# hellosunking/Microcket

Hardware: AMD Instinct MI355X
Metric: read-pairs/sec through sam2pairs+dedup (150 bp PE, hg38 names, SAM text resident in HBM) (higher is better)
Workload: dtype u8; 1 GPU; C2: 100 M 150 bp PE Micro-C read pairs, hg38, one MI355X -- 100000000 synthetic 150 bp PE read pairs per GPU, hg38 chromosome names, 1 lane(s), unc mode, sam=no, seed 20260105, one step = one pass over the whole resident data set + duplicate marking of the reported pairs on (chr1,pos1,chr2,pos2,strands) + per-chromosome-pair counts; preset=C2, pairs_per_gpu=100000001, sam_bytes_per_gpu=94584442002, block_groups=2097152, blocks=48, parallelism=shard1: independent read-group shards, no data-path collective

## Files before the change

### microcket_amd/build.py

```python
import os
import shutil
import subprocess
import sys

HERE = os.path.dirname(os.path.abspath(__file__))
ROOT = os.path.dirname(HERE)
CSRC = os.path.join(HERE, "csrc")
LIB = os.path.join(HERE, "libmkt_hip.so")
EXE = os.path.join(HERE, "bin", "sam2pairs")
ARCH = "gfx950"


def _newer(target, sources):
    if not os.path.exists(target):
        return True
    t = os.path.getmtime(target)
    return any(os.path.getmtime(s) > t for s in sources)


def _run(cmd, **kw):
    print("+", " ".join(cmd), flush=True)
    subprocess.check_call(cmd, **kw)


# ... 134 lines not shown


PAIRSCMP = os.path.join(HERE, "bin", "pairscmp")


def build_pairscmp(force=False):
    src = os.path.join(CSRC, "pairscmp_main.cpp")
    if force or _newer(PAIRSCMP, [src, LIB] + _headers()):
        os.makedirs(os.path.dirname(PAIRSCMP), exist_ok=True)
        _run(["g++", "-O2", "-std=c++17", "-Wall", src, "-o", PAIRSCMP, "-L" + HERE, "-lmkt_hip",
              "-Wl,-rpath,$ORIGIN/..", "-Wl,-rpath,/opt/rocm/lib", "-Wl,-rpath-link,/opt/rocm/lib"])
    return PAIRSCMP


PAIRSBGZ = os.path.join(HERE, "bin", "pairsbgz")


def build_pairsbgz(force=False):
    src = os.path.join(CSRC, "pairsbgz_main.cpp")
    if force or _newer(PAIRSBGZ, [src, LIB] + _headers()):
        os.makedirs(os.path.dirname(PAIRSBGZ), exist_ok=True)
        _run(["g++", "-O2", "-std=c++17", "-Wall", src, "-o", PAIRSBGZ, "-L" + HERE, "-lmkt_hip",
              "-Wl,-rpath,$ORIGIN/..", "-Wl,-rpath,/opt/rocm/lib", "-Wl,-rpath-link,/opt/rocm/lib"])
    return PAIRSBGZ


PAIRSGUNZIP = os.path.join(HERE, "bin", "pairsgunzip")


def build_pairsgunzip(force=False):
    src = os.path.join(CSRC, "pairsgunzip_main.cpp")
    if force or _newer(PAIRSGUNZIP, [src, LIB] + _headers()):
        os.makedirs(os.path.dirname(PAIRSGUNZIP), exist_ok=True)
        _run(["g++", "-O2", "-std=c++17", "-Wall", src, "-o", PAIRSGUNZIP, "-L" + HERE, "-lmkt_hip",
              "-Wl,-rpath,$ORIGIN/..", "-Wl,-rpath,/opt/rocm/lib", "-Wl,-rpath-link,/opt/rocm/lib"])
    return PAIRSGUNZIP


PAIRSQUERY = os.path.join(HERE, "bin", "pairsquery")


def build_pairsquery(force=False):
    src = os.path.join(CSRC, "pairsquery_main.cpp")
    if force or _newer(PAIRSQUERY, [src, LIB] + _headers()):
        os.makedirs(os.path.dirname(PAIRSQUERY), exist_ok=True)
        _run(["g++", "-O2", "-std=c++17", "-Wall", src, "-o", PAIRSQUERY, "-L" + HERE, "-lmkt_hip",
              "-Wl,-rpath,$ORIGIN/..", "-Wl,-rpath,/opt/rocm/lib", "-Wl,-rpath-link,/opt/rocm/lib"])
    return PAIRSQUERY


BAM2SAM = os.path.join(HERE, "bin", "bam2sam")


def build_bam2sam(force=False):
    src = os.path.join(CSRC, "bam2sam_main.cpp")
    if force or _newer(BAM2SAM, [src, LIB] + _headers()):
        os.makedirs(os.path.dirname(BAM2SAM), exist_ok=True)
        _run(["g++", "-O2", "-std=c++17", "-Wall", src, "-o", BAM2SAM, "-L" + HERE, "-lmkt_hip",
              "-Wl,-rpath,$ORIGIN/..", "-Wl,-rpath,/opt/rocm/lib", "-Wl,-rpath-link,/opt/rocm/lib"])
    return BAM2SAM


MAKESTAT = os.path.join(HERE, "bin", "makestat")


def build_makestat(force=False):
    src = os.path.join(CSRC, "makestat_main.cpp")
    if force or _newer(MAKESTAT, [src]):
        os.makedirs(os.path.dirname(MAKESTAT), exist_ok=True)
        _run(["g++", "-O2", "-std=c++17", "-Wall", src, "-o", MAKESTAT])
    return MAKESTAT


def build_oracle():
    _run(["make", "-s", "-C", os.path.join(ROOT, "oracle")])


def build_emit_parts():
    out = os.path.join(ROOT, "tests", "host", "_build")
    os.makedirs(out, exist_ok=True)
    src = os.path.join(ROOT, "tests", "host", "emit_parts.cpp")
    made = []
    for name, extra in (("emit_parts", ()), ("emit_parts_san", ("-fsanitize=address,undefined", "-fno-sanitize-recover=all", "-fno-omit-frame-pointer"))):
        exe = os.path.join(out, name)
        if os.path.exists(src) and _newer(exe, [src] + _headers()):
            _run(["g++", "-O1", "-g", "-std=c++17", "-Wall", *extra, "-o", exe, src])
        made.append(exe)
    return made


def build_test_tools():
    out = os.path.join(ROOT, "tests", "host", "_build")
    os.makedirs(out, exist_ok=True)
    emul = os.path.join(out, "libmkt_emul.so")
    src = os.path.join(ROOT, "tests", "host", "tile_emul.cpp")
    if _newer(emul, [src] + _headers()):
        _run(["g++", "-O1", "-g", "-std=c++17", "-Wall", "-fPIC", "-shared", "-o", emul, src])
    dzc = os.path.join(out, "deflate_codes")
    dsrc = os.path.join(ROOT, "tests", "host", "deflate_codes.cpp")
    if os.path.exists(dsrc) and _newer(dzc, [dsrc, os.path.join(CSRC, "mkt_deflate_codes.h")]):
        _run(["g++", "-O1", "-g", "-std=c++17", "-Wall", "-o", dzc, dsrc])
    sth = os.path.join(out, "stitch_thresholds")
    tsrc = os.path.join(ROOT, "tests", "host", "stitch_thresholds.cpp")
    if os.path.exists(tsrc) and _newer(sth, [tsrc, os.path.join(CSRC, "mkt_stitch.h"), os.path.join(ROOT, "include", "mkt.h")]):
        _run(["g++", "-O1", "-g", "-std=c++17", "-Wall", "-o", sth, tsrc])
    dbc = os.path.join(out, "devbuf_check")
    bsrc = os.path.join(ROOT, "tests", "host", "devbuf_check.cpp")
    if os.path.exists(bsrc) and _newer(dbc, [bsrc, os.path.join(CSRC, "mkt_devbuf.h")]):
        _run([hipcc(), f"--offload-arch={ARCH}", "-O1", "-g", "-std=c++17", "-Wall", "-Wl,-rpath,/opt/rocm/lib", "-o", dbc, bsrc])
    vsrc = os.path.join(ROOT, "tests", "host", "viewpoint_host.cpp")
    for name, extra in (("viewpoint_host", ()), ("viewpoint_host_san", ("-fsanitize=address,undefined", "-fno-sanitize-recover=all", "-fno-omit-frame-pointer"))):
        vph = os.path.join(out, name)
        if os.path.exists(vsrc) and _newer(vph, [vsrc, os.path.join(CSRC, "mkt_viewpoint.h"), os.path.join(ROOT, "include", "mkt.h")]):
            _run(["g++", "-O1", "-g", "-std=c++17", "-Wall", *extra, "-o", vph, vsrc])
    csrc = os.path.join(ROOT, "tests", "host", "chunked_file.cpp")
    for name, extra in (("chunked_file", ()), ("chunked_file_san", ("-fsanitize=address,undefined", "-fno-sanitize-recover=all", "-fno-omit-frame-pointer"))):
        chf = os.path.join(out, name)
        if os.path.exists(csrc) and _newer(chf, [csrc, os.path.join(CSRC, "mkt_chunked_file.h")]):
            _run(["g++", "-O1", "-g", "-std=c++17", "-Wall", *extra, "-o", chf, csrc])
    psrc = os.path.join(ROOT, "tests", "host", "paircmp_host.cpp")
    for name, extra in (("paircmp_host", ()), ("paircmp_host_san", ("-fsanitize=address,undefined", "-fno-sanitize-recover=all", "-fno-omit-frame-pointer"))):
        pch = os.path.join(out, name)
        if os.path.exists(psrc) and _newer(pch, [psrc, os.path.join(CSRC, "mkt_paircmp.h"), os.path.join(ROOT, "include", "mkt.h")]):
            _run(["g++", "-O1", "-g", "-std=c++17", "-Wall", *extra, "-o", pch, psrc])
    xsrc = os.path.join(ROOT, "tests", "host", "px2_host.cpp")
    for name, extra in (("px2_host", ()), ("px2_host_san", ("-fsanitize=address,undefined", "-fno-sanitize-recover=all", "-fno-omit-frame-pointer"))):
        pxh = os.path.join(out, name)
        if os.path.exists(xsrc) and _newer(pxh, [xsrc, os.path.join(CSRC, "mkt_px2.h")]):
            _run(["g++", "-O1", "-g", "-std=c++17", "-Wall", *extra, "-o", pxh, xsrc])
    isrc = os.path.join(ROOT, "tests", "host", "inflate_host.cpp")
    for name, extra in (("inflate_host", ()), ("inflate_host_san", ("-fsanitize=address,undefined", "-fno-sanitize-recover=all", "-fno-omit-frame-pointer"))):
        ifh = os.path.join(out, name)
        if os.path.exists(isrc) and _newer(ifh, [isrc, os.path.join(CSRC, "mkt_inflate.h")]):
            _run(["g++", "-O1", "-g", "-std=c++17", "-Wall", *extra, "-o", ifh, isrc])
    qsrc = os.path.join(ROOT, "tests", "host", "pairsquery_host.cpp")
    for name, extra in (("pairsquery_host", ()), ("pairsquery_host_san", ("-fsanitize=address,undefined", "-fno-sanitize-recover=all", "-fno-omit-frame-pointer"))):
        pqh = os.path.join(out, name)
        if os.path.exists(qsrc) and _newer(pqh, [qsrc, os.path.join(CSRC, "mkt_px2query.h"), os.path.join(CSRC, "mkt_inflate.h")]):
            _run(["g++", "-O1", "-g", "-std=c++17", "-Wall", *extra, "-o", pqh, qsrc])
    bsrc2 = os.path.join(ROOT, "tests", "host", "bamtext_host.cpp")
    for name, extra in (("bamtext_host", ()), ("bamtext_host_san", ("-fsanitize=address,undefined", "-fno-sanitize-recover=all", "-fno-omit-frame-pointer"))):
        bth = os.path.join(out, name)
        if os.path.exists(bsrc2) and _newer(bth, [bsrc2, os.path.join(CSRC, "mkt_bamtext.h")]):
            _run(["g++", "-O1", "-g", "-std=c++17", "-Wall", *extra, "-o", bth, bsrc2])
    build_emit_parts()
    tout = os.path.join(ROOT, "tools", "_build")
    os.makedirs(tout, exist_ok=True)
    synth = os.path.join(tout, "synth_sam")
    ssrc = os.path.join(ROOT, "tools", "synth_sam.cpp")
    if _newer(synth, [ssrc, os.path.join(CSRC, "mkt_synth.h")]):
        _run(["g++", "-O2", "-std=c++17", "-Wall", "-o", synth, ssrc])


def build_all(force=False, extras=True):
    build_lib(force)
    build_exe(force)
    build_pairsort(force)
    build_krmdup(force)
    build_stitch(force)
    build_sam2bam(force)
    build_pairs2matrix(force)
    build_pairscmp(force)
    build_pairsbgz(force)
    build_pairsgunzip(force)
    build_pairsquery(force)
    build_bam2sam(force)
    build_makestat(force)
    if extras:
        build_oracle()
        build_test_tools()


if __name__ == "__main__":
    build_all(force="--force" in sys.argv, extras="--all" in sys.argv or True)
```

### microcket_amd/csrc/mkt_fast.h

```cpp
#pragma once
#include "mkt_tile.h"

namespace mkt {

#if defined(MKT_LEAN_GEOM)
constexpr int kLeanGeom[4] = {MKT_LEAN_GEOM};
constexpr int kLeanTile = kLeanGeom[0], kLeanHB = kLeanGeom[1], kLeanHF = kLeanGeom[2], kLeanLCAP = kLeanGeom[3];
#else
constexpr int kLeanTile = 49152, kLeanHB = 3072, kLeanHF = 4096, kLeanLCAP = 168;
#endif
constexpr int kMidTile = 32768, kMidHB = 2048, kMidHF = 3072, kMidLCAP = 160;
constexpr int kDenseTile = 16384, kDenseHB = 1024, kDenseHF = 2048, kDenseLCAP = 160;
constexpr int kLeanLinesTarget = 126;

constexpr double kLeanHaloBackLines = 7.5, kLeanHaloFwdLines = 8.75;
MKT_HD TileDims lean_dims(double avg) {
    if (avg < 48.0) avg = 48.0;
    if (avg > 4096.0) avg = 4096.0;
    auto r16 = [](double x) { return ((uint32_t)x + 15u) & ~15u; };
    TileDims d;
    d.hb = r16(kLeanHaloBackLines * avg); d.hf = r16(kLeanHaloFwdLines * avg);
    if (d.hb < 256u) d.hb = 256u;
    if (d.hb > (uint32_t)kLeanHB) d.hb = (uint32_t)kLeanHB;
    if (d.hf < 512u) d.hf = 512u;
// ... 17 lines not shown
    static constexpr int HCH = 8, HEADB = HCH * 16;
    static constexpr int HSTRIDE = HEADB + 4;
    static constexpr int HW = LCAP_ * HSTRIDE;
    static_assert(TILE_ % 16 == 0 && HB_ % 16 == 0 && HF_ % 16 == 0, "16-byte vector staging");
    static_assert(W < 65536, "window-relative offsets are 16 bit");
    static_assert(LCAP_ <= 255, "line / group ordinals are 8 bit");
    static_assert(LCAP_ * 132 < 65536, "head-store offsets are 16 bit");
};

enum { AB_LCAP = 1, AB_LONG, AB_TAB, AB_PREV_WS, AB_PREV_HEAD, AB_NO_PREV, AB_OPEN_GROUP, AB_LAST_LINE, AB_GCAP, AB_PAIR_BYTES, AB_SHORT_LINE };

constexpr uint8_t LB_EMIT = 8;

template <class Cfg>
struct FastState {
    alignas(16) uint8_t win[Cfg::HW + 16];
    struct Recs {
        struct { uint32_t pos[Cfg::LCAP], lclip[Cfg::LCAP], rclip[Cfg::LCAP], mappable[Cfg::LCAP], right0[Cfg::LCAP], left1[Cfg::LCAP], right1[Cfg::LCAP]; } f;
    } rc;
    uint16_t hv16[Cfg::LCAP];
    uint16_t off16[Cfg::LCAP];
    uint16_t goff[Cfg::LCAP];
    uint16_t flag[Cfg::LCAP];
    uint8_t qn_off[Cfg::LCAP], qn_len[Cfg::LCAP], rn_off[Cfg::LCAP], rn_len[Cfg::LCAP], segCnt[Cfg::LCAP], bits[Cfg::LCAP];
    union alignas(16) Phase {
        struct {
            uint64_t hitmap[Cfg::HMW + 1];
            alignas(8) uint16_t hmask[Cfg::LCAP][Cfg::HCH];
        } m;
        struct {
            uint32_t g_info[Cfg::LCAP], g_slen[Cfg::LCAP];
            uint32_t x_sam[Cfg::LCAP];
            uint16_t g_plen[Cfg::LCAP], x_pair[Cfg::LCAP];
            uint8_t x_grp[Cfg::LCAP], x_sc[Cfg::LCAP], x_emit[Cfg::LCAP], em_idx[Cfg::LCAP], g_slot[Cfg::LCAP];
            uint32_t l_posA[Cfg::GCAP], l_posB[Cfg::GCAP];
            uint16_t l_qa[Cfg::GCAP], l_ca[Cfg::GCAP], l_cb[Cfg::GCAP];
            uint16_t l_e0[Cfg::GCAP], l_e1[Cfg::GCAP], l_e2[Cfg::GCAP], l_e3[Cfg::GCAP];
            uint64_t l_litA[Cfg::GCAP][2], l_litB[Cfg::GCAP][2];
        } g;
    } u;
    uint64_t m_surv[4], m_eqp[4], m_r1[4], m_r2[4], m_start[4], m_emit[4];
    uint64_t cc[64];
    uint32_t NL, first_idx, end_idx, abn, last_line_end, nslot, c_t0, c_t1;
    uint32_t cnt[C_COUNT];
    TileSums sums, base;
    uint32_t region_pair0, region_sam0, region_id;
};

template <class Cfg> MKT_HD TileGeom fast_geom(uint32_t tile, uint32_t n) { return tile_geom(tile, n, cfg_dims<Cfg>()); }
template <class Cfg> MKT_HD TextView fast_view(const FastState<Cfg>& st, const uint8_t* text, uint32_t n, const TileGeom& G) {
    TextView tv;
    (void)G;
    tv.g = text; tv.n = n; tv.win = st.win; tv.w0 = 0; tv.wlen = Cfg::HW; tv.nlm = nullptr; tv.wsm = nullptr;
    return tv;
}
template <class Cfg> MKT_HD void fast_init(FastState<Cfg>& st, uint32_t k) { if (k < 64u) st.cc[k] = 0; }
template <class Cfg> MKT_HD uint32_t fast_chr_slot(FastState<Cfg>& st, ChrTab* tab, const TextView& tv, uint32_t off, uint32_t len, uint32_t* err) {
    static_assert(kChrSlots <= 8192, "slot in 13 bits");
    if (len == 0u || len > 6u) return chr_slot(tab, tv, off, len, err);
    const uint64_t name = ((uint64_t)win_load4(tv, off) | ((uint64_t)win_load4(tv, off + 4u) << 32)) & ((1ull << (8u * len)) - 1ull);
    const uint32_t idx = (uint32_t)((name * 0x9E3779B1ull) >> 30) & 63u;
    const uint64_t e0 = st.cc[idx], e1 = st.cc[idx ^ 1u];
    if ((e0 >> 63) && (e0 & 0xFFFFFFFFFFFFull) == name) return (uint32_t)(e0 >> 48) & 8191u;
    if ((e1 >> 63) && (e1 & 0xFFFFFFFFFFFFull) == name) return (uint32_t)(e1 >> 48) & 8191u;
    const uint32_t s = chr_slot(tab, tv, off, len, err);
    st.cc[(e0 >> 63) && !(e1 >> 63) ? (idx ^ 1u) : idx] = name | ((uint64_t)s << 48) | (1ull << 63);
    return s;
}
template <class Cfg> MKT_HD void fast_reset(FastState<Cfg>& st) {
    st.NL = 0; st.first_idx = 0; st.end_idx = 0; st.abn = 0; st.last_line_end = kUnknown; st.nslot = 0; st.c_t0 = 0; st.c_t1 = 0;
    for (int k = 0; k < 4; ++k) st.m_emit[k] = 0;
    st.region_pair0 = 0; st.region_sam0 = 0; st.region_id = 0;
    for (int k = 0; k < (int)C_COUNT; ++k) st.cnt[k] = 0;
}
template <class Cfg> MKT_HD uint32_t fast_nle(const FastState<Cfg>& st) {
    return (st.NL && (st.bits[st.NL - 1] & LB_CUT)) ? st.NL - 1u : st.NL;
}
template <class Cfg> MKT_HD uint32_t fast_line_end(const FastState<Cfg>& st, const TileGeom& G, uint32_t i) {
    return i + 1 < st.NL ? G.w0 + st.goff[i + 1] - 1u : st.last_line_end;
}

template <class Cfg> MKT_HD void fast_head_ws(const FastState<Cfg>& st, uint32_t i, uint64_t& ws0, uint64_t& ws1) {
    const uint64_t* row = reinterpret_cast<const uint64_t*>(st.u.m.hmask[i]);
    const uint64_t A = row[0], B = row[1];
    const uint32_t sh = (uint32_t)st.off16[i] - mul24(i, (uint32_t)Cfg::HSTRIDE);
    ws0 = sh ? ((A >> sh) | (B << (64u - sh))) : A;
    ws1 = B >> sh;
}
template <class Cfg> MKT_HD void fast_head_chunk_ref(FastState<Cfg>& st, const uint8_t* text, uint32_t n, const TileGeom& G, uint32_t i, uint32_t c) {
    const uint32_t r0 = 16u * ((uint32_t)st.hv16[i] + c);
    uint32_t m = 0;
    for (uint32_t b = 0; b < 16u; ++b) {
        const uint64_t g = (uint64_t)G.w0 + r0 + b;
        const uint8_t ch = g < n ? text[g] : 0;
        st.win[i * Cfg::HSTRIDE + 16u * c + b] = ch;
        if (g < n && ch <= 0x20u) m |= 1u << b;
    }
    st.u.m.hmask[i][c] = (uint16_t)m;
}

MKT_HD uint32_t nl_flags_exact(uint32_t x) {
    const uint32_t y = (x ^ 0x0A0A0A0Au), z = y & 0x7F7F7F7Fu;
    return ~((z + 0x7F7F7F7Fu) | y | 0x7F7F7F7Fu);
}
template <class Cfg> MKT_HD uint32_t fast_row_start(const FastState<Cfg>& st, const TileGeom& G, uint32_t i, bool* multi) {
    *multi = false;
    if (i == 0u && G.w0 == 0u) return 0u;
    const uint32_t* row = reinterpret_cast<const uint32_t*>(&st.win[mul24(i, (uint32_t)Cfg::HSTRIDE)]);
    const uint32_t f0 = nl_flags_exact(row[0]), f1 = nl_flags_exact(row[1]), f2 = nl_flags_exact(row[2]), f3 = nl_flags_exact(row[3]);
    const uint32_t m = (f0 >> 7) | (f1 >> 6) | (f2 >> 5) | (f3 >> 4);
    *multi = (m & (m - 1u)) != 0u;
    const uint32_t p = f0 ? (ctz32(f0) >> 3) : (f1 ? 4u + (ctz32(f1) >> 3) : (f2 ? 8u + (ctz32(f2) >> 3) : 12u + (ctz32(f3 | 0x80000000u) >> 3)));
    return p + 1u;
}

enum { LP_OK = 1, LP_NOREC = 2, LP_LONG = 0, LP_ODD = -1 };

MKT_HD uint32_t dec4(uint32_t w, bool& ok) {
    const uint32_t d = w ^ 0x30303030u;
    if (((d + 0x76767676u) | d) & 0x80808080u) ok = false;
    const uint32_t x = (d << 3) + (d << 1) + (d >> 8);
    return mul24(x & 0xFFu, 100u) + ((x >> 16) & 0xFFu);
}
MKT_HD uint32_t lean_uint4(const TextView& tv, uint32_t a, uint32_t len, bool& ok) {
    const uint32_t sh = 8u * (4u - len);
    const uint32_t w = (win_load4(tv, a) << sh) | (0x30303030u & ((1u << sh) - 1u));
    return dec4(w, ok);
}
MKT_HD uint32_t lean_uint12(const TextView& tv, uint32_t e, uint32_t len, bool& ok) {
    const uint32_t* w = reinterpret_cast<const uint32_t*>(tv.win);
    const uint32_t a = e - 12u, k = a >> 2, sh = a & 3u;
    const uint32_t q0 = w[k], q1 = w[k + 1], q2 = w[k + 2], q3 = w[k + 3];
    uint32_t x0, x1, x2;
#if defined(__HIP_DEVICE_COMPILE__)
    x0 = __builtin_amdgcn_alignbyte(q1, q0, sh); x1 = __builtin_amdgcn_alignbyte(q2, q1, sh); x2 = __builtin_amdgcn_alignbyte(q3, q2, sh);
#else
    x0 = sh ? ((q0 >> (8u * sh)) | (q1 << (32u - 8u * sh))) : q0;
    x1 = sh ? ((q1 >> (8u * sh)) | (q2 << (32u - 8u * sh))) : q1;
    x2 = sh ? ((q2 >> (8u * sh)) | (q3 << (32u - 8u * sh))) : q2;
#endif
    const uint32_t lead = 12u - len;
    const uint32_t n0 = lead < 4u ? lead : 4u, n1 = lead < 4u ? 0u : (lead < 8u ? lead - 4u : 4u), n2 = lead < 8u ? 0u : lead - 8u;
    const uint32_t m0 = n0 >= 4u ? 0xFFFFFFFFu : ((1u << (8u * n0)) - 1u), m1 = n1 >= 4u ? 0xFFFFFFFFu : ((1u << (8u * n1)) - 1u),
                   m2 = (1u << (8u * n2)) - 1u;
    x0 = (x0 & ~m0) | (0x30303030u & m0); x1 = (x1 & ~m1) | (0x30303030u & m1); x2 = (x2 & ~m2) | (0x30303030u & m2);
    const uint32_t A = dec4(x0, ok), B = dec4(x1, ok), C = dec4(x2, ok);
    const uint64_t v = (uint64_t)A * 100000000ull + (uint64_t)(mul24(B, 10000u) + C);
    if (v > 0xFFFFFFFFull) ok = false;
    return (uint32_t)v;
}
MKT_HD bool lean_eq(const TextView& tv, uint32_t a, uint32_t b, uint32_t len) {
    const uint32_t* w = reinterpret_cast<const uint32_t*>(tv.win);
    const uint32_t ka = a >> 2, sa = a & 3u, kb = b >> 2, sb = b & 3u;
    uint32_t acc = 0;
    for (uint32_t i = 0; i < len; i += 8u) {
        const uint32_t j = i >> 2;
        const uint32_t a0 = w[ka + j], a1 = w[ka + j + 1], a2 = w[ka + j + 2], b0 = w[kb + j], b1 = w[kb + j + 1], b2 = w[kb + j + 2];
        uint32_t x0, x1, y0, y1;
#if defined(__HIP_DEVICE_COMPILE__)
        x0 = __builtin_amdgcn_alignbyte(a1, a0, sa); x1 = __builtin_amdgcn_alignbyte(a2, a1, sa);
        y0 = __builtin_amdgcn_alignbyte(b1, b0, sb); y1 = __builtin_amdgcn_alignbyte(b2, b1, sb);
#else
        x0 = sa ? ((a0 >> (8u * sa)) | (a1 << (32u - 8u * sa))) : a0; x1 = sa ? ((a1 >> (8u * sa)) | (a2 << (32u - 8u * sa))) : a1;
        y0 = sb ? ((b0 >> (8u * sb)) | (b1 << (32u - 8u * sb))) : b0; y1 = sb ? ((b1 >> (8u * sb)) | (b2 << (32u - 8u * sb))) : b1;
#endif
        uint32_t d0 = x0 ^ y0, d1 = x1 ^ y1;
        const uint32_t rem = len - i;
        if (rem < 4u) { d0 &= (1u << (8u * rem)) - 1u; d1 = 0; }
        else if (rem < 8u) { d1 &= (1u << (8u * (rem - 4u))) - 1u; }
        acc |= d0 | d1;
    }
    return acc == 0u;
}

struct LeanCigar {
    int32_t index, cur, lastRight;
    bool bad;
};
MKT_HD void lean_cigar_op(Rec& r, LeanCigar& w, uint32_t c, int32_t v, bool last) {
    const bool hs = c == 'H' || c == 'S', m = c == 'M', d = c == 'D', n = c == 'N', known = hs || m || d || n || c == 'I';
    const bool live = !w.bad;
    const bool first = w.index == 0;
    if (live && (!known || (hs && !last && !first))) w.bad = true;
    const bool go = live && !w.bad;
    const bool md = go && (m || d), nn = go && n;
    if (go && hs && last) r.rclip = v;
    if (go && hs && !last && first) r.lclip = v;
    if (go && m) r.mappable += v;
    w.cur += (md || nn) ? v : 0;
    w.lastRight = md ? w.cur - 1 : (nn ? 0 : w.lastRight);
    if (md && first) r.right0 = w.lastRight;
    if (md && w.index == 1) r.right1 = w.lastRight;
    if (nn && first) { r.left1 = w.cur; r.right1 = 0; }
    w.index += nn ? 1 : 0;
}

MKT_HD int parse_record_lean(const TextView& tv, uint32_t off, const Params& P, Rec& r, uint64_t sp0, uint64_t sp1, uint32_t reach) {
    if (reach < 64u) sp0 |= 1ull << reach; else if (reach < 128u) sp1 |= 1ull << (reach - 64u);
    uint32_t p[6];
    if (sp0 == 0ull) return LP_LONG;
    p[0] = ctz64(sp0);
    if (p[0] >= 63u) return LP_LONG;
    const uint32_t b0 = p[0] + 1u;
    uint64_t rest = (sp0 >> b0) | (sp1 << (64u - b0));
#if defined(__HIP_DEVICE_COMPILE__)
#pragma unroll
#endif
    for (int k = 1; k < 6; ++k) {
        p[k] = rest ? b0 + ctz64(rest) : 0xFFFFu;
        rest &= rest - 1ull;
    }
    uint32_t c[6];
#if defined(__HIP_DEVICE_COMPILE__)
#pragma unroll
#endif
    for (int k = 0; k < 6; ++k) c[k] = tv.win[off + (p[k] == 0xFFFFu ? 0u : p[k])];
    uint32_t miss = 0, adj = 0, nl = 0, odd = 0;
#if defined(__HIP_DEVICE_COMPILE__)
#pragma unroll
#endif
    for (int k = 0; k < 6; ++k) {
        const uint32_t prev = k ? p[k - 1] + 1u : 0u;
        miss |= (p[k] == 0xFFFFu ? 1u : 0u) << k;
        adj |= (p[k] == prev ? 1u : 0u) << k;
        nl |= ((p[k] == reach || c[k] == '\n') ? 1u : 0u) << k;
        odd |= (c[k] != '\t' ? 1u : 0u) << k;
    }
    const uint32_t ev = (miss | adj | nl | odd) & 0x3Fu;
    if (ev) {
        const uint32_t f = 1u << ctz32(ev);
        if (miss & f) return LP_LONG;
        if (adj & f) return (nl & f) ? LP_NOREC : LP_ODD;
        if (nl & f) { if (f != 32u) return LP_NOREC; }
        else return LP_ODD;
    }
    bool ok = tv.win[off] != '@';
    r.qn_off = 0; r.qn_len = p[0];
    r.rn_off = p[1] + 1u; r.rn_len = p[2] - p[1] - 1u;
    const uint32_t fl_len = p[1] - p[0] - 1u, pos_len = p[3] - p[2] - 1u, mq_len = p[4] - p[3] - 1u;
    if (pos_len > 10u || p[3] < 12u) return LP_ODD;
    r.pos = lean_uint12(tv, off + p[3], pos_len, ok);
    if (fl_len <= 4u) r.flag = lean_uint4(tv, off + p[0] + 1u, fl_len, ok);
    else if (fl_len > 10u || p[1] < 12u) return LP_ODD;
    else r.flag = lean_uint12(tv, off + p[1], fl_len, ok);
    if (mq_len <= 4u) r.mapq = lean_uint4(tv, off + p[3] + 1u, mq_len, ok);
    else if (mq_len > 10u) return LP_ODD;
    else r.mapq = lean_uint12(tv, off + p[4], mq_len, ok);
    const uint32_t cs = off + p[4] + 1u, clen = p[5] - p[4] - 1u;
    if (clen > 32u || p[4] < 12u) return LP_ODD;
    uint32_t dig = 0;
    for (uint32_t k = 0; k < clen; k += 4u) dig |= digit_bits4(win_load4(tv, cs + k)) << k;
    const uint32_t cmask = clen >= 32u ? 0xFFFFFFFFu : ((1u << clen) - 1u);
    uint32_t ops = ~dig & cmask;
    LeanCigar w;
    w.index = 0; w.cur = (int32_t)r.pos; w.lastRight = 0; w.bad = false;
    r.left0 = (int32_t)r.pos;
    uint32_t run0 = 0;
    bool odd_count = false;
    while (ops) {
        const uint32_t q = ctz32(ops);
        ops &= ops - 1u;
        const uint32_t L = q - run0;
        bool vok = true;
        uint32_t value;
        if (L <= 4u) {
            const uint32_t sh = 8u * (4u - L);
            const uint32_t x = win_load4(tv, cs + q - 4u);
            value = L ? dec4((x & ~((1u << sh) - 1u)) | (0x30303030u & ((1u << sh) - 1u)), vok) : 0u;
        } else if (L <= 9u) value = lean_uint12(tv, cs + q, L, vok);
        else { value = 0; odd_count = true; }
        lean_cigar_op(r, w, tv.win[cs + q], (int32_t)value, q + 1u == clen);
        run0 = q + 1u;
    }
    if (odd_count) return LP_ODD;
    if (!w.bad && w.lastRight != 0) { r.segCnt = w.index + 1; r.rightLast = w.lastRight; }
    r.survive = ok && !(r.flag & 0x700u) && r.mapq >= P.min_mapq;
    return LP_OK;
}

template <class Cfg> MKT_HD void fast_parse(FastState<Cfg>& st, const TextView& tv, const Params& P, const TileGeom& G, uint32_t i) {
    bool multi;
    const uint32_t soff = fast_row_start(st, G, i, &multi);
    if (multi) st.abn = AB_SHORT_LINE;
    const uint32_t goff = 16u * (uint32_t)st.hv16[i] + soff;
    const uint32_t off = mul24(i, (uint32_t)Cfg::HSTRIDE) + soff;
    st.goff[i] = (uint16_t)goff;
    st.off16[i] = (uint16_t)off;
    const uint32_t gl = G.w0 + goff;
    if (gl >= G.w1) {
        st.bits[i] = LB_CUT;
        if (i + 1u != st.NL) st.abn = AB_SHORT_LINE;
        return;
    }
    Rec r;
    uint64_t ws0, ws1;
    fast_head_ws(st, i, ws0, ws1);
    rec_clear(r, off);
    const int pf = parse_record_lean(tv, off, P, r, ws0, ws1, tv.n - gl);
    if (pf == LP_LONG || pf == LP_ODD) {
        if (gl >= G.t1 && i + 1 == st.NL && G.w1 < tv.n) st.bits[i] = LB_CUT;
        else { st.bits[i] = 0; st.abn = pf == LP_LONG ? AB_LONG : AB_TAB; }
        return;
    }
    st.rc.f.pos[i] = r.pos; st.rc.f.lclip[i] = (uint32_t)r.lclip; st.rc.f.rclip[i] = (uint32_t)r.rclip; st.rc.f.mappable[i] = (uint32_t)r.mappable;
    st.rc.f.right0[i] = (uint32_t)r.right0; st.rc.f.left1[i] = (uint32_t)r.left1; st.rc.f.right1[i] = (uint32_t)r.right1;
    st.flag[i] = (uint16_t)(r.flag & 0xFFFFu);
    st.qn_off[i] = (uint8_t)r.qn_off; st.qn_len[i] = (uint8_t)r.qn_len; st.rn_off[i] = (uint8_t)r.rn_off; st.rn_len[i] = (uint8_t)r.rn_len;
    st.segCnt[i] = (uint8_t)(r.segCnt > 4 ? 4 : r.segCnt);
    uint8_t b = r.survive ? LB_SURVIVE : 0;
    if (i > 0 && pf == LP_OK) {
        bool pm;
        const uint32_t psoff = fast_row_start(st, G, i - 1u, &pm);
        const uint32_t poff = mul24(i - 1u, (uint32_t)Cfg::HSTRIDE) + psoff;
        const uint32_t ql = r.qn_len;
        if (ql + 1u > (uint32_t)Cfg::HEADB - psoff || ql > 100u) st.abn = AB_PREV_HEAD;
        else if (lean_eq(tv, off, poff, ql + 1u)) b |= LB_EQPREV;
    }
    st.bits[i] = b;
}

MKT_HD bool mask_bit(const uint64_t* m, uint32_t i) { return (m[i >> 6] >> (i & 63u)) & 1ull; }
MKT_HD uint64_t mask_range(uint32_t w, uint32_t lo, uint32_t hi) {
    const uint32_t b = w << 6;
    if (hi <= b || lo >= b + 64u) return 0ull;
    const uint32_t l = lo > b ? lo - b : 0u, h = hi < b + 64u ? hi - b : 64u;
    const uint64_t up = h >= 64u ? ~0ull : ((1ull << h) - 1ull);
    return up & ~((1ull << l) - 1ull);
}
MKT_HD uint64_t mask_win(const uint64_t* m, uint32_t start) {
    const uint32_t w = start >> 6, s = start & 63u;
    uint64_t x = m[w] >> s;
    if (s && w < 3u) x |= m[w + 1u] << (64u - s);
    return x;
}
MKT_HD uint64_t mask_win_back(const uint64_t* m, uint32_t i) {
    return i >= 63u ? mask_win(m, i - 63u) : (m[0] << (63u - i));
}
MKT_HD uint32_t mask_next(const uint64_t* m, uint32_t from, uint32_t limit) {
    for (uint32_t w = from >> 6; (w << 6) < limit && w < 4u; ++w) {
        const uint64_t x = m[w] & mask_range(w, from, limit);
        if (x) return (w << 6) + ctz64(x);
    }
    return limit;
}
template <class Cfg> MKT_HD void fast_build_masks(FastState<Cfg>& st) {
    for (int k = 0; k < 4; ++k) st.m_surv[k] = st.m_eqp[k] = st.m_r1[k] = st.m_r2[k] = 0;
    for (uint32_t i = 0; i < st.NL; ++i) {
        const uint64_t bit = 1ull << (i & 63u);
        if (st.bits[i] & LB_SURVIVE) st.m_surv[i >> 6] |= bit;
        if (st.bits[i] & LB_EQPREV) st.m_eqp[i >> 6] |= bit;
        if ((st.bits[i] & LB_SURVIVE) && (st.flag[i] & 64u)) st.m_r1[i >> 6] |= bit;
        if ((st.bits[i] & LB_SURVIVE) && !(st.flag[i] & 64u) && (st.flag[i] & 128u)) st.m_r2[i >> 6] |= bit;
    }
}

template <class Cfg> MKT_HD bool fast_is_start(FastState<Cfg>& st, const TextView& tv, const TileGeom& G, uint32_t i) {
    const uint64_t sv = mask_win_back(st.m_surv, i) & ~(1ull << 63);
    if (!sv) {
        if (G.w0 == 0 && i < 64u) return true;
        st.abn = AB_NO_PREV;
        return false;
    }
    const uint32_t d = clz64(sv), p = i - d;
    if (((~mask_win_back(st.m_eqp, i)) >> (64u - d)) == 0ull) return false;
    if (d == 1u) return true;
    return !text_eq<true>(tv, (uint32_t)st.off16[i] + st.qn_off[i], st.qn_len[i], (uint32_t)st.off16[p] + st.qn_off[p], st.qn_len[p]);
}

template <class Cfg> MKT_HD Seg fast_seg(const FastState<Cfg>& st, uint32_t idx) {
    Seg s;
    s.segCnt = st.segCnt[idx]; s.lclip = (int32_t)st.rc.f.lclip[idx]; s.rclip = (int32_t)st.rc.f.rclip[idx]; s.mappable = (int32_t)st.rc.f.mappable[idx];
    s.left0 = (int32_t)st.rc.f.pos[idx]; s.left1 = (int32_t)st.rc.f.left1[idx]; s.right0 = (int32_t)st.rc.f.right0[idx]; s.right1 = (int32_t)st.rc.f.right1[idx];
    s.rightLast = s.segCnt == 2 ? s.right1 : s.right0;
    s.flag = st.flag[idx]; s.pos = st.rc.f.pos[idx];
    s.chr_off = (uint32_t)st.off16[idx] + st.rn_off[idx]; s.chr_len = st.rn_len[idx];
    {
        const uint32_t* w = reinterpret_cast<const uint32_t*>(st.win);
        const uint32_t k = s.chr_off >> 2, sh = s.chr_off & 3u;
        const uint32_t q0 = w[k], q1 = w[k + 1], q2 = w[k + 2];
        uint32_t x0, x1;
#if defined(__HIP_DEVICE_COMPILE__)
        x0 = __builtin_amdgcn_alignbyte(q1, q0, sh); x1 = __builtin_amdgcn_alignbyte(q2, q1, sh);
#else
        x0 = sh ? ((q0 >> (8u * sh)) | (q1 << (32u - 8u * sh))) : q0; x1 = sh ? ((q1 >> (8u * sh)) | (q2 << (32u - 8u * sh))) : q1;
#endif
        const uint32_t n = s.chr_len;
        if (n < 4u) { x0 &= (1u << (8u * n)) - 1u; x1 = 0; }
        else if (n < 8u) x1 &= (1u << (8u * (n - 4u))) - 1u;
        s.chr_key = ((uint64_t)bswap32(x0) << 32) | bswap32(x1);
    }
    return s;
}

template <class Cfg> MKT_HD void fast_group(FastState<Cfg>& st, const TextView& tv, const Params& P, const TileGeom& G, uint32_t i) {
    auto& g = st.u.g;
    g.g_info[i] = 0; g.g_plen[i] = 0; g.g_slen[i] = 0;
// ... 216 lines not shown
```

### microcket_amd/csrc/mkt_kernels.hip

```cpp
#include <hip/hip_runtime.h>
#include <type_traits>
#include "mkt_launch.h"

namespace mkt {

constexpr int NT = 256;
constexpr uint64_t FLAG_AGG = 1ull << 62, FLAG_PREFIX = 2ull << 62, PAYLOAD = (1ull << 62) - 1;
constexpr uint32_t LOOKBACK_SPIN_LIMIT = 1u << 22;

struct ScanScratch { uint64_t a[NT / 64], b[NT / 64]; };

#if defined(MKT_STAMPS)
#define STAMP_DECL() unsigned long long stamp_prev_ = 0, stamp_first_ = 0, stamp_acc_[16] = {0, 0, 0, 0, 0, 0, 0, 0, 0, 0, 0, 0, 0, 0, 0, 0}
#define STAMP(k)                                                                        \
    do {                                                                                \
        if (tid == 0 && a.stamps) {                                                     \
            const unsigned long long now_ = __builtin_amdgcn_s_memtime();               \
            if ((k) > 0) stamp_acc_[(k)] += now_ - stamp_prev_;                         \
            else if (!stamp_first_) stamp_first_ = __builtin_amdgcn_s_memrealtime();   \
            stamp_prev_ = now_;                                                         \
        }                                                                               \
    } while (0)
#define STAMP_SPAN(t0_)                                                                 \
    do {                                                                                \
// ... 521 lines not shown
        int tid = tid0;
        asm volatile("" : "+v"(tid));
        if (tid == 0) fast_reset(st);
        STAMP(0);
        const TileGeom G = tile_geom(t, n, a.dims);
        const TextView tv = fast_view(st, a.text, n, G);

        const uint32_t wave = (uint32_t)__builtin_amdgcn_readfirstlane(tid >> 6);
        if (!scanned) fast_scan<Cfg, NWV>(a, t, s_hit[cur], wave, 0u, own(wave, NWV, lpt_all), tid & 63);
        scanned = false;
        __syncthreads();
        STAMP(1);
        STOP_AFTER(1)

        if (tid < 64) {
            static_assert(Cfg::HMW <= 64, "one bitmap word per lane of one wave");
            uint64_t m = (uint32_t)tid < ((G.w1 - G.w0 + 1023u) >> 10) ? s_hit[cur][tid] : 0ull;
            const uint32_t cnt = (uint32_t)__popcll(m);
            const uint32_t inc = wave_iscan32(cnt);
            const uint32_t total = (uint32_t)__builtin_amdgcn_readlane((int)inc, 63);
            const uint32_t lead = G.w0 == 0 ? 1u : 0u;
            const uint32_t NLt = total + lead;
            if (NLt > (uint32_t)Cfg::LCAP) {
                if (tid == 0) { st.abn = AB_LCAP; st.NL = 0; }
            } else {
                uint32_t idx = inc - cnt + lead;
                while (m) {
                    st.hv16[idx++] = (uint16_t)(((uint32_t)tid << 6) + (uint32_t)__builtin_ctzll(m));
                    m &= m - 1ull;
                }
                if (tid == 0) {
                    if (lead) st.hv16[0] = 0;
                    st.NL = NLt; st.first_idx = NLt; st.end_idx = NLt;
                    st.last_line_end = G.w1 >= n ? n : kUnknown;
                }
            }
        }
        __syncthreads();
        const uint32_t NL = st.NL;
        STAMP(2);
        STOP_AFTER(2)
        {
            constexpr int HPT = (Cfg::LCAP * Cfg::HCH + NTW - 1) / NTW;
            auto heads = [&](auto edge_c) {
                constexpr bool EDGE = decltype(edge_c)::value;
                uint4 q[HPT];
#pragma unroll
                for (int k = 0; k < HPT; ++k) {
                    const uint32_t it = (uint32_t)tid + (uint32_t)k * NTW;
                    q[k] = make_uint4(0, 0, 0, 0);
                    if (it < NL * (uint32_t)Cfg::HCH) {
                        const uint32_t i = it / (uint32_t)Cfg::HCH, c = it % (uint32_t)Cfg::HCH;
                        const uint32_t g0 = G.w0 + (((uint32_t)st.hv16[i] + c) << 4);
                        if (!EDGE || g0 < n) q[k] = *reinterpret_cast<const uint4*>(a.text + g0);
                    }
                }
#pragma unroll
                for (int k = 0; k < HPT; ++k) {
                    const uint32_t it = (uint32_t)tid + (uint32_t)k * NTW;
                    if (it >= NL * (uint32_t)Cfg::HCH) continue;
                    const uint32_t i = it / (uint32_t)Cfg::HCH, c = it % (uint32_t)Cfg::HCH;
                    uint4 x = q[k];
                    uint32_t keep = 16u;
                    if (EDGE) {
                        const uint32_t g0 = G.w0 + (((uint32_t)st.hv16[i] + c) << 4);
                        keep = g0 >= n ? 0u : (n - g0 < 16u ? n - g0 : 16u);
                        if (keep != 0u && keep < 16u) {
                            uint32_t* w = reinterpret_cast<uint32_t*>(&x);
#pragma unroll
                            for (int d = 0; d < 4; ++d) {
                                const uint32_t lo = (uint32_t)d * 4u;
                                w[d] = keep >= lo + 4u ? w[d] : (keep > lo ? (w[d] & ((1u << ((keep - lo) * 8u)) - 1u)) : 0u);
                            }
                        }
                    }
                    {
                        uint32_t* row = reinterpret_cast<uint32_t*>(&st.win[mul24(i, (uint32_t)Cfg::HSTRIDE) + (c << 4)]);
                        row[0] = x.x; row[1] = x.y; row[2] = x.z; row[3] = x.w;
                    }
                    uint32_t m = pack16(sep_flags(x.x), sep_flags(x.y), sep_flags(x.z), sep_flags(x.w));
                    if (EDGE && keep < 16u) m &= (1u << keep) - 1u;
                    st.u.m.hmask[i][c] = (uint16_t)m;
                }
            };
            if ((uint64_t)G.w1 + 16u * ((uint32_t)Cfg::HCH + 2u) > (uint64_t)n) heads(std::true_type{});
            else heads(std::false_type{});
        }
        __syncthreads();
        STAMP(9);
        STOP_AFTER(9)

        const uint32_t ltid = (uint32_t)tid;
        const uint32_t rr_id = ((uint32_t)tid >> 6) < (uint32_t)RR ? ((uint32_t)tid & 63u) * RR + ((uint32_t)tid >> 6) : 0xFFFFFFu;
        {
            const uint32_t i = ltid;
            uint32_t lb = 0, fl = 0;
            if (i < NL) { fast_parse(st, tv, P, G, i); lb = st.bits[i]; fl = st.flag[i]; }
            const bool sv = (lb & LB_SURVIVE) != 0;
            const uint64_t b_s = __ballot(sv), b_e = __ballot((lb & LB_EQPREV) != 0);
            const uint64_t b_1 = __ballot(sv && (fl & 64u)), b_2 = __ballot(sv && !(fl & 64u) && (fl & 128u));
            const uint32_t gs = i < NL ? (uint32_t)st.goff[i] : 0u;
            const uint64_t b_t0 = __ballot(i < NL && G.w0 + gs >= G.t0), b_t1 = __ballot(i < NL && G.w0 + gs >= G.t1);
            if ((tid & 63) == 0) {
                const uint32_t w = ltid >> 6; st.m_surv[w] = b_s; st.m_eqp[w] = b_e; st.m_r1[w] = b_1; st.m_r2[w] = b_2;
                if (b_t0) atomicAdd(&st.c_t0, (uint32_t)__popcll(b_t0));
                if (b_t1) atomicAdd(&st.c_t1, (uint32_t)__popcll(b_t1));
            }
            if (NTW < 256 && tid < 4 && tid >= NTW / 64) { st.m_surv[tid] = 0; st.m_eqp[tid] = 0; st.m_r1[tid] = 0; st.m_r2[tid] = 0; st.m_start[tid] = 0; }
        }
        if (NSW && wave >= (uint32_t)(NWV - NSW)) {
            const uint32_t nxt = next_of(t, cur);
            if (nxt < a.ntiles)
                fast_scan<Cfg, (NSW ? NSW : 1)>(a, nxt, s_hit[cur ^ 1u], wave - (uint32_t)(NWV - NSW), 0u, own(wave - (uint32_t)(NWV - NSW), NSW, lpt_a), tid & 63);
        }
        __syncthreads();
        STAMP(3);
        STOP_AFTER(3)
        const uint32_t NLe = fast_nle(st);
        const uint32_t first_idx = NL - st.c_t0 < NLe ? NL - st.c_t0 : NLe;
        const uint32_t end_idx = NL - st.c_t1 < NLe ? NL - st.c_t1 : NLe;
        {
            const uint32_t i = ltid;
            bool s0 = false;
            if (!st.abn && i >= first_idx && i < NLe && mask_bit(st.m_surv, i)) s0 = fast_is_start(st, tv, G, i);
            const uint64_t b = __ballot(s0);
            if ((tid & 63) == 0) st.m_start[ltid >> 6] = b;
        }
        __syncthreads();
        STAMP(10);
#if defined(MKT_STAMPS)
        if (a.debug_stop == 10) {
            if (a.out.sam && !st.abn) for (uint32_t i = first_idx + (uint32_t)tid; i < end_idx; i += NTW) {
                const uint4 r0 = make_uint4(st.rc.f.pos[i], st.rc.f.lclip[i] | (st.rc.f.rclip[i] << 16), st.rc.f.mappable[i] | ((uint32_t)st.flag[i] << 16), st.rc.f.right0[i]);
                const uint4 r1 = make_uint4(st.rc.f.left1[i], st.rc.f.right1[i], G.w0 + st.goff[i], st.qn_len[i] | ((uint32_t)st.rn_off[i] << 8) | ((uint32_t)st.rn_len[i] << 16) | ((uint32_t)st.bits[i] << 24));
                uint4* d = reinterpret_cast<uint4*>(a.out.sam + ((size_t)t * Cfg::LCAP + i) * 32u);
                if (((size_t)t * Cfg::LCAP + i) * 32u + 32u <= a.out.sam_cap) { d[0] = r0; d[1] = r1; }
            }
            const uint32_t nxt = next_of(t, cur);
            if (NSW && wave >= (uint32_t)(NWV - NSW) && nxt < a.ntiles)
                fast_scan<Cfg, (NSW ? NSW : 1)>(a, nxt, s_hit[cur ^ 1u], wave - (uint32_t)(NWV - NSW), lpt_a, own(wave - (uint32_t)(NWV - NSW), NSW, lpt_sw), tid & 63);
            scanned = NSW && nxt < a.ntiles; cur ^= 1u;
            __syncthreads();
            continue;
        }
#endif
        if (!st.abn) for (uint32_t i = first_idx + rr_id; i < end_idx; i += 64 * RR) fast_group(st, tv, P, G, i);
        {
            const uint32_t nxt = next_of(t, cur);
            const bool draw = nxt < a.ntiles && nxt + gdim >= a.fast_dyn0;
            uint32_t tk = 0;
            if (draw && ticket_lane) tk = atomicAdd(a.fast_ticket, 1u);
            if (NSW && wave >= (uint32_t)(NWV - NSW) && nxt < a.ntiles)
                fast_scan<Cfg, (NSW ? NSW : 1)>(a, nxt, s_hit[cur ^ 1u], wave - (uint32_t)(NWV - NSW), lpt_a, own(wave - (uint32_t)(NWV - NSW), NSW, lpt_sw), tid & 63);
            if (draw && ticket_lane) s_next[cur ^ 1u] = a.fast_dyn0 + tk;
            scanned = NSW && nxt < a.ntiles; cur ^= 1u;
        }
        __syncthreads();
        STAMP(4);
        STOP_AFTER(4)
        STAMP(5);

        {
            auto& g = st.u.g;
            const uint32_t i = first_idx + tid;
            uint32_t cc = 0, cp = 0, cs = 0;
            uint32_t info = 0;
// ... 794 lines not shown
```

Measured before the change: 2.311 billion read-pairs/s.

## Precompute line starts and pre-shift head masks during head loading; streamline lean_eq

```diff
diff --git a/microcket_amd/build.py b/microcket_amd/build.py
--- a/microcket_amd/build.py
+++ b/microcket_amd/build.py
@@ -240,6 +240,19 @@
     src = os.path.join(ROOT, "tests", "host", "emit_parts.cpp")
     made = []
     for name, extra in (("emit_parts", ()), ("emit_parts_san", ("-fsanitize=address,undefined", "-fno-sanitize-recover=all", "-fno-omit-frame-pointer"))):
+        exe = os.path.join(out, name)
+        if os.path.exists(src) and _newer(exe, [src] + _headers()):
+            _run(["g++", "-O1", "-g", "-std=c++17", "-Wall", *extra, "-o", exe, src])
+        made.append(exe)
+    return made
+
+
+def build_parse_chain():
+    out = os.path.join(ROOT, "tests", "host", "_build")
+    os.makedirs(out, exist_ok=True)
+    src = os.path.join(ROOT, "tests", "host", "parse_chain.cpp")
+    made = []
+    for name, extra in (("parse_chain", ()), ("parse_chain_san", ("-fsanitize=address,undefined", "-fno-sanitize-recover=all", "-fno-omit-frame-pointer"))):
         exe = os.path.join(out, name)
         if os.path.exists(src) and _newer(exe, [src] + _headers()):
             _run(["g++", "-O1", "-g", "-std=c++17", "-Wall", *extra, "-o", exe, src])
@@ -302,6 +315,7 @@
         if os.path.exists(bsrc2) and _newer(bth, [bsrc2, os.path.join(CSRC, "mkt_bamtext.h")]):
             _run(["g++", "-O1", "-g", "-std=c++17", "-Wall", *extra, "-o", bth, bsrc2])
     build_emit_parts()
+    build_parse_chain()
     tout = os.path.join(ROOT, "tools", "_build")
     os.makedirs(tout, exist_ok=True)
     synth = os.path.join(tout, "synth_sam")
diff --git a/microcket_amd/csrc/mkt_fast.h b/microcket_amd/csrc/mkt_fast.h
--- a/microcket_amd/csrc/mkt_fast.h
+++ b/microcket_amd/csrc/mkt_fast.h
@@ -123,11 +123,9 @@
 
 template <class Cfg> MKT_HD void fast_head_ws(const FastState<Cfg>& st, uint32_t i, uint64_t& ws0, uint64_t& ws1) {
     const uint64_t* row = reinterpret_cast<const uint64_t*>(st.u.m.hmask[i]);
-    const uint64_t A = row[0], B = row[1];
-    const uint32_t sh = (uint32_t)st.off16[i] - mul24(i, (uint32_t)Cfg::HSTRIDE);
-    ws0 = sh ? ((A >> sh) | (B << (64u - sh))) : A;
-    ws1 = B >> sh;
-}
+    ws0 = row[0]; ws1 = row[1];
+}
+template <class Cfg> MKT_HD void fast_head_line(FastState<Cfg>& st, const TileGeom& G, uint32_t i);
 template <class Cfg> MKT_HD void fast_head_chunk_ref(FastState<Cfg>& st, const uint8_t* text, uint32_t n, const TileGeom& G, uint32_t i, uint32_t c) {
     const uint32_t r0 = 16u * ((uint32_t)st.hv16[i] + c);
     uint32_t m = 0;
@@ -138,6 +136,7 @@
         if (g < n && ch <= 0x20u) m |= 1u << b;
     }
     st.u.m.hmask[i][c] = (uint16_t)m;
+    if (c + 1u == (uint32_t)Cfg::HCH) fast_head_line(st, G, i);
 }
 
 MKT_HD uint32_t nl_flags_exact(uint32_t x) {
@@ -153,6 +152,18 @@
     *multi = (m & (m - 1u)) != 0u;
     const uint32_t p = f0 ? (ctz32(f0) >> 3) : (f1 ? 4u + (ctz32(f1) >> 3) : (f2 ? 8u + (ctz32(f2) >> 3) : 12u + (ctz32(f3 | 0x80000000u) >> 3)));
     return p + 1u;
+}
+constexpr uint8_t LB_HEAD_SHORT = 1;
+template <class Cfg> MKT_HD void fast_head_line(FastState<Cfg>& st, const TileGeom& G, uint32_t i) {
+    bool multi;
+    const uint32_t sh = fast_row_start(st, G, i, &multi);
+    st.goff[i] = (uint16_t)(16u * (uint32_t)st.hv16[i] + sh);
+    st.off16[i] = (uint16_t)(mul24(i, (uint32_t)Cfg::HSTRIDE) + sh);
+    st.bits[i] = multi ? LB_HEAD_SHORT : 0;
+    uint64_t* row = reinterpret_cast<uint64_t*>(st.u.m.hmask[i]);
+    const uint64_t A = row[0], B = row[1];
+    row[0] = sh ? ((A >> sh) | (B << (64u - sh))) : A;
+    row[1] = B >> sh;
 }
 
 enum { LP_OK = 1, LP_NOREC = 2, LP_LONG = 0, LP_ODD = -1 };
@@ -190,28 +201,34 @@
     if (v > 0xFFFFFFFFull) ok = false;
     return (uint32_t)v;
 }
+MKT_HD uint32_t lean_align(uint32_t hi, uint32_t lo, uint32_t s) {
+#if defined(__HIP_DEVICE_COMPILE__)
+    return __builtin_amdgcn_alignbyte(hi, lo, s);
+#else
+    return s ? ((lo >> (8u * s)) | (hi << (32u - 8u * s))) : lo;
+#endif
+}
 MKT_HD bool lean_eq(const TextView& tv, uint32_t a, uint32_t b, uint32_t len) {
     const uint32_t* w = reinterpret_cast<const uint32_t*>(tv.win);
-    const uint32_t ka = a >> 2, sa = a & 3u, kb = b >> 2, sb = b & 3u;
+    const uint32_t sa = a & 3u, sb = b & 3u;
+    uint32_t ka = a >> 2, kb = b >> 2, rem = len;
+    uint32_t a0 = w[ka], b0 = w[kb];
     uint32_t acc = 0;
-    for (uint32_t i = 0; i < len; i += 8u) {
-        const uint32_t j = i >> 2;
-        const uint32_t a0 = w[ka + j], a1 = w[ka + j + 1], a2 = w[ka + j + 2], b0 = w[kb + j], b1 = w[kb + j + 1], b2 = w[kb + j + 2];
-        uint32_t x0, x1, y0, y1;
-#if defined(__HIP_DEVICE_COMPILE__)
-        x0 = __builtin_amdgcn_alignbyte(a1, a0, sa); x1 = __builtin_amdgcn_alignbyte(a2, a1, sa);
-        y0 = __builtin_amdgcn_alignbyte(b1, b0, sb); y1 = __builtin_amdgcn_alignbyte(b2, b1, sb);
-#else
-        x0 = sa ? ((a0 >> (8u * sa)) | (a1 << (32u - 8u * sa))) : a0; x1 = sa ? ((a1 >> (8u * sa)) | (a2 << (32u - 8u * sa))) : a1;
-        y0 = sb ? ((b0 >> (8u * sb)) | (b1 << (32u - 8u * sb))) : b0; y1 = sb ? ((b1 >> (8u * sb)) | (b2 << (32u - 8u * sb))) : b1;
-#endif
-        uint32_t d0 = x0 ^ y0, d1 = x1 ^ y1;
-        const uint32_t rem = len - i;
-        if (rem < 4u) { d0 &= (1u << (8u * rem)) - 1u; d1 = 0; }
-        else if (rem < 8u) { d1 &= (1u << (8u * (rem - 4u))) - 1u; }
-        acc |= d0 | d1;
-    }
-    return acc == 0u;
+    for (; rem > 16u; rem -= 16u) {
+        const uint32_t a1 = w[ka + 1], a2 = w[ka + 2], a3 = w[ka + 3], a4 = w[ka + 4];
+        const uint32_t b1 = w[kb + 1], b2 = w[kb + 2], b3 = w[kb + 3], b4 = w[kb + 4];
+        acc |= (lean_align(a1, a0, sa) ^ lean_align(b1, b0, sb)) | (lean_align(a2, a1, sa) ^ lean_align(b2, b1, sb));
+        acc |= (lean_align(a3, a2, sa) ^ lean_align(b3, b2, sb)) | (lean_align(a4, a3, sa) ^ lean_align(b4, b3, sb));
+        a0 = a4; b0 = b4; ka += 4u; kb += 4u;
+    }
+    const uint32_t far = rem > 8u ? 1u : 0u;
+    const uint32_t a1 = w[ka + 1], a2 = w[ka + 2], a3 = w[ka + 2 + far], a4 = w[ka + 2 + 2u * far];
+    const uint32_t b1 = w[kb + 1], b2 = w[kb + 2], b3 = w[kb + 2 + far], b4 = w[kb + 2 + 2u * far];
+    const uint64_t d0 = (uint64_t)(lean_align(a1, a0, sa) ^ lean_align(b1, b0, sb)) | ((uint64_t)(lean_align(a2, a1, sa) ^ lean_align(b2, b1, sb)) << 32);
+    const uint64_t d1 = (uint64_t)(lean_align(a3, a2, sa) ^ lean_align(b3, b2, sb)) | ((uint64_t)(lean_align(a4, a3, sa) ^ lean_align(b4, b3, sb)) << 32);
+    const uint32_t n0 = far ? 8u : rem;
+    const uint64_t t0 = d0 << (64u - 8u * n0), t1 = far ? d1 << (128u - 8u * rem) : 0ull;
+    return (t0 | t1 | (uint64_t)acc) == 0ull;
 }
 
 struct LeanCigar {
@@ -320,14 +337,9 @@
 }
 
 template <class Cfg> MKT_HD void fast_parse(FastState<Cfg>& st, const TextView& tv, const Params& P, const TileGeom& G, uint32_t i) {
-    bool multi;
-    const uint32_t soff = fast_row_start(st, G, i, &multi);
-    if (multi) st.abn = AB_SHORT_LINE;
-    const uint32_t goff = 16u * (uint32_t)st.hv16[i] + soff;
-    const uint32_t off = mul24(i, (uint32_t)Cfg::HSTRIDE) + soff;
-    st.goff[i] = (uint16_t)goff;
-    st.off16[i] = (uint16_t)off;
-    const uint32_t gl = G.w0 + goff;
+    const uint32_t off = st.off16[i];
+    if (st.bits[i]) st.abn = AB_SHORT_LINE;
+    const uint32_t gl = G.w0 + (uint32_t)st.goff[i];
     if (gl >= G.w1) {
         st.bits[i] = LB_CUT;
         if (i + 1u != st.NL) st.abn = AB_SHORT_LINE;
@@ -350,9 +362,8 @@
     st.segCnt[i] = (uint8_t)(r.segCnt > 4 ? 4 : r.segCnt);
     uint8_t b = r.survive ? LB_SURVIVE : 0;
     if (i > 0 && pf == LP_OK) {
-        bool pm;
-        const uint32_t psoff = fast_row_start(st, G, i - 1u, &pm);
-        const uint32_t poff = mul24(i - 1u, (uint32_t)Cfg::HSTRIDE) + psoff;
+        const uint32_t poff = st.off16[i - 1u];
+        const uint32_t psoff = poff - mul24(i - 1u, (uint32_t)Cfg::HSTRIDE);
         const uint32_t ql = r.qn_len;
         if (ql + 1u > (uint32_t)Cfg::HEADB - psoff || ql > 100u) st.abn = AB_PREV_HEAD;
         else if (lean_eq(tv, off, poff, ql + 1u)) b |= LB_EQPREV;
diff --git a/microcket_amd/csrc/mkt_kernels.hip b/microcket_amd/csrc/mkt_kernels.hip
--- a/microcket_amd/csrc/mkt_kernels.hip
+++ b/microcket_amd/csrc/mkt_kernels.hip
@@ -627,6 +627,16 @@
                     if (EDGE && keep < 16u) m &= (1u << keep) - 1u;
                     st.u.m.hmask[i][c] = (uint16_t)m;
                 }
+                constexpr uint32_t LPW = 64u / (uint32_t)Cfg::HCH;
+                static_assert(64 % Cfg::HCH == 0 && NTW % Cfg::HCH == 0 && HPT * (64 / Cfg::HCH) <= 64, "the lines of a wave's chunks, a lane each");
+                __builtin_amdgcn_fence(__ATOMIC_RELEASE, "wavefront");
+                __builtin_amdgcn_wave_barrier();
+                __builtin_amdgcn_fence(__ATOMIC_ACQUIRE, "wavefront");
+                {
+                    const uint32_t l = (uint32_t)tid & 63u;
+                    const uint32_t i = (((uint32_t)tid >> 6) * LPW) + (l / LPW) * (uint32_t)(NTW / Cfg::HCH) + (l % LPW);
+                    if (l < (uint32_t)HPT * LPW && i < NL) fast_head_line(st, G, i);
+                }
             };
             if ((uint64_t)G.w1 + 16u * ((uint32_t)Cfg::HCH + 2u) > (uint64_t)n) heads(std::true_type{});
             else heads(std::false_type{});
```

Result: faster. 2.366 billion read-pairs/s (median of 6 runs) (+2.4%).
